# CrystalSixone/VLN-MAGIC

Hardware: AMD Instinct MI355X
Metric: trajectory-steps/sec (whole node), MAGIC-S R2R pretrain (higher is better)
Workload: dtype bf16

## Files before the change

include/magic_hip.h:

```cpp
#ifndef MAGIC_HIP_H
#define MAGIC_HIP_H
#ifdef __cplusplus
extern "C" {
#endif

#define MAGIC_OK 0
#define MAGIC_ERR_ARG (-1)
#define MAGIC_ERR_LAUNCH (-2)
#define MAGIC_ERR_UNSUPPORTED (-3)

int magic_abi_version(void);
int magic_build_id(char* out, int len);
int magic_device_info(int* cu_count, int* clock_khz, char* arch, int arch_len);

int magic_gemm(int dtype, int layout, int batch, int nh, int M, int N, int K,
               const void* A, int lda, long long sAb, long long sAh,
               const void* B, int ldb, long long sBb, long long sBh,
               void* C, int ldc, long long sCb, long long sCh, int c_f32, int accumulate,
               const float* bias, int epilogue, const void* aux, int ldaux,
               const void* residual, int ldr, void* C2, int ldc2,
               float alpha, int splitk, float* bias_grad, void* stream);
int magic_gemm_set_big(int mode);
#define MAGIC_GEMM_FORM_PLAIN 0x1
#define MAGIC_GEMM_FORM_XCD 0x2
// ... 148 lines not shown
int magic_lndot_fwd(int dtype, int M, int H, const void* Y, const float* gamma, const float* beta, float eps,
                    const float* w2, const float* b2, float* logit, void* stream);
int magic_lndot_bwd_blocks(int M);
int magic_lndot_bwd(int dtype, int M, int H, const void* Y, const float* gamma, const float* beta, float eps,
                    const float* w2, const float* dlogit, void* dZ, float* dgamma, float* dbeta, float* dw2, float* db2,
                    float* part, void* stream);

int magic_ce_rows(int dtype, int M, int N, const void* logits, int ld, const int* labels, int ignore_index,
                  float coef, const float* row_w, float* loss_row, void* dlogits, int ldd, int accumulate,
                  float* w_out, float w_rate, void* stream);
int magic_softkl_rows(int dtype, int M, int N, const void* logits, int ld, const float* targets, int ldt, float coef,
                      const float* row_w , float* loss_row, void* dlogits, int ldd,
                      void* stream);

int magic_kd_rows(int M, int N, const float* s, const float* t, int ld, float temperature, const float* w, float norm,
                  float coef, const float* coef_dev, float* loss_row, float* ds, int accumulate, void* stream);
int magic_mse(int dtype, int g_f32, long long outer, long long inner, const void* s, long long s_stride, const void* t,
              long long t_stride, const float* w, long long rows_per_w, float norm, float coef, const float* coef_dev, float* loss, void* ds,
              long long g_stride, int accumulate, void* stream);
typedef struct {
  int g_f32; long long outer, inner; const void* s; long long s_stride; const void* t; long long t_stride;
  const float* w; long long rows_per_w; float norm, coef; const float* coef_dev; float* loss; void* ds; long long g_stride; int accumulate;
  const int* valid_dev; const float* norm_dev; long long valid_mod;
} magic_mse_desc;
int magic_mse_multi(int dtype, int n, const magic_mse_desc* d, void* stream);
int magic_kd_emb_supported(int dtype, int Hs, int Ht);
int magic_kd_emb(int dtype, int n, const magic_mse_desc* d, int Hs, int Ht, const int* M, const void* const* W, const float* const* b,
                 void* const* d_acc, void* stream);
int magic_cfp_loss(int dtype, int B, int H, const void* a0, const void* a1, const void* a2, const void* txt, float temperature, float coef,
                   float* rows, void* d0, void* d1, void* d2, void* dtxt, float* part, int* counter, void* stream);

int magic_mlm_eval_supported(int dtype, int H);
int magic_mlm_eval_ws_need(int dtype, int nm, int V, int H);
int magic_mlm_eval(int dtype, int nm, int V, int H, const void* hm, const void* W, int ldw, const float* bias,
                   const int* labels, int ignore_index, void* ws, float* loss_row, int* hit_row, void* stream);
int magic_eval_rows(int dtype, int M, int N, const void* logits, int ld, const int* labels, int ignore_index,
                    const float* targets, int ldt, float* loss_row, int* hit_row, void* stream);
int magic_cfp_eval(int dtype, int B, int H, const void* a, const void* txt, float temperature,
                   float* loss_row, int* hit_row, void* stream);
int magic_eval_accum(int M, const float* loss_row, const int* hit_row, void* acc, int slot, void* stream);

int magic_csr_gather(int dtype, int n_out, int H, const void* src, const int* ptr, const int* idx, const float* w,
                     void* out, int accumulate, void* stream);
int magic_pano_fuse_fwd(int dtype, int N, int V, int H, const void* x, const int* lens, const float* wf, const float* bf,
                        void* fused, float* probs, const void* P, int nh, int inner, float* pmean, void* stream);
typedef struct {
  int B, K, Vp, use_gate;
  const float *g_raw, *l_raw, *fuse_raw; const unsigned char *gmask, *lmask; const int* fsrc; const unsigned char* bwmask;
// ... 131 lines not shown
```

vln-magic_amd/csrc/loss.hip:

```cpp
#include "common.hpp"
#include <cstdint>

static const float* g_seed_scale = nullptr;
const float* seed_scale_get() { return g_seed_scale; }
extern "C" int magic_seed_scale(const float* scale_dev) { g_seed_scale = scale_dev; return MAGIC_OK; }

template <typename T>
__global__ __launch_bounds__(256) void ce_rows_kernel(int M, int N, const T* logits, int ld, const int* labels, int ignore_index,
                                                      float coef, const float* row_w, float* loss_row, T* dlogits, int ldd,
                                                      int accumulate, float* w_out, float w_rate, const float* ss) {
  __shared__ float red[8];
  if (ss) coef *= ss[0];
  const int row = blockIdx.x, tid = threadIdx.x, lane = tid & 63, wid = tid >> 6;
  const T* x = logits + (long long)row * ld;
  const int lab = labels[row];
  const bool ignored = (lab == ignore_index) || lab < 0 || lab >= N;
  const float xl = ignored ? 0.f : to_f(x[lab]);
  float mx = -3.0e38f;
  for (int c = tid; c < N; c += 256) mx = fmaxf(mx, to_f(x[c]));
  mx = wave_max(mx);
  if (lane == 0) red[wid] = mx;
  __syncthreads();
  mx = fmaxf(fmaxf(red[0], red[1]), fmaxf(red[2], red[3]));
  __syncthreads();
// ... 191 lines not shown
  if (coef_dev) coef *= coef_dev[0];
  if (ss) coef *= ss[0];
  const long long total = outer * inner;
  float acc = 0.f;
  for (long long i = (long long)blockIdx.x * 256 + threadIdx.x; i < total; i += (long long)gridDim.x * 256) {
    const long long o = i / inner, r = i % inner;
    const float d = to_f(s[o * s_stride + r]) - to_f(t[o * t_stride + r]);
    const float wv = w ? w[o / rows_per_w] : 1.f;
    acc += wv * d * d;
    if (ds) {
      float g = 2.f * coef * norm * wv * d;
      G* p = ds + o * g_stride + r;
      if (accumulate) g += to_f(*p);
      *p = from_f<G>(g);
    }
  }
  acc = wave_sum(acc);
  if ((threadIdx.x & 63) == 0) red[threadIdx.x >> 6] = acc;
  __syncthreads();
  if (threadIdx.x == 0 && loss) atomicAdd(loss, (red[0] + red[1] + red[2] + red[3]) * norm);
}

#define MSE_MAX 10
struct MseMulti { magic_mse_desc d[MSE_MAX]; int start[MSE_MAX + 1]; int vec[MSE_MAX]; int n; const float* ss; };

#define MSE_NT 1024
template <typename T, typename G>
__device__ __forceinline__ void mse_body(const magic_mse_desc& p, int bid, int nblk, float* red, const float* ss) {
  float coef = p.coef;
  if (p.coef_dev) coef *= p.coef_dev[0];
  if (ss) coef *= ss[0];
  const T* s = (const T*)p.s; const T* t = (const T*)p.t; G* ds = (G*)p.ds;
  const long long total = p.outer * p.inner;
  const long long vo = p.valid_dev ? p.valid_dev[0] : p.outer, vi = p.valid_dev ? p.valid_dev[1] : p.inner;
  const float nrm = p.norm * (p.norm_dev ? p.norm_dev[0] : 1.f);
  float acc = 0.f;
  for (long long i = (long long)bid * MSE_NT + threadIdx.x; i < total; i += (long long)nblk * MSE_NT) {
    const long long o = i / p.inner, r = i % p.inner;
    const bool ok = o < vo && (p.valid_mod > 0 ? r % p.valid_mod : r) < vi;
    const float d = ok ? to_f(s[o * p.s_stride + r]) - to_f(t[o * p.t_stride + r]) : 0.f;
    const float wv = p.w ? p.w[o / p.rows_per_w] : 1.f;
    acc += wv * d * d;
    if (ds) {
      float g = 2.f * coef * nrm * wv * d;
      G* q = ds + o * p.g_stride + r;
      if (p.accumulate) g += to_f(*q);
      *q = from_f<G>(g);
    }
  }
  acc = wave_sum(acc);
  if ((threadIdx.x & 63) == 0) red[threadIdx.x >> 6] = acc;
  __syncthreads();
  if (threadIdx.x == 0 && p.loss) {
    float v = 0.f;
    for (int w = 0; w < MSE_NT / 64; ++w) v += red[w];
    atomicAdd(p.loss, v * nrm);
  }
}

template <typename Hh, typename G>
__device__ __forceinline__ void mse_body_v8(const magic_mse_desc& p, int bid, int nblk, float* red, const float* ss) {
  float coef = p.coef;
  if (p.coef_dev) coef *= p.coef_dev[0];
  if (ss) coef *= ss[0];
  const Hh* s = (const Hh*)p.s; const Hh* t = (const Hh*)p.t; G* ds = (G*)p.ds;
  const unsigned in8 = (unsigned)(p.inner >> 3), tot8 = (unsigned)p.outer * in8, rpw = (unsigned)p.rows_per_w;
  const unsigned stride = (unsigned)nblk * MSE_NT;
  const unsigned vo = p.valid_dev ? (unsigned)p.valid_dev[0] : (unsigned)p.outer, vi = p.valid_dev ? (unsigned)p.valid_dev[1] : (unsigned)p.inner;
  const float nrm = p.norm * (p.norm_dev ? p.norm_dev[0] : 1.f);
  const float c2 = 2.f * coef * nrm;
// ... 9 lines not shown
      ok[u] = i < tot8;
      const unsigned ii = ok[u] ? i : i0;
      o[u] = ii / in8; r[u] = (ii - o[u] * in8) << 3;
      sv[u] = *(const h16x8<Hh>*)(s + (long long)o[u] * p.s_stride + r[u]);
      tv[u] = *(const h16x8<Hh>*)(t + (long long)o[u] * p.t_stride + r[u]);
    }
#pragma unroll
    for (int u = 0; u < 2; ++u) {
      if (!ok[u]) continue;
      const float wv = p.w ? p.w[o[u] / rpw] : 1.f;
      float d[8];
      float a = 0.f;
      const unsigned rm = vm ? r[u] % vm : r[u];
#pragma unroll
      for (int e = 0; e < 8; ++e) { d[e] = (o[u] < vo && rm + e < vi) ? (float)sv[u][e] - (float)tv[u][e] : 0.f; a += d[e] * d[e]; }
      acc += wv * a;
      if (ds) {
        G* q = ds + (long long)o[u] * p.g_stride + r[u];
        const float cw = c2 * wv;
        if constexpr (sizeof(G) == 4) {
          f32x4 g0, g1;
#pragma unroll
          for (int e = 0; e < 4; ++e) { g0[e] = cw * d[e]; g1[e] = cw * d[4 + e]; }
          if (p.accumulate) { g0 += *(const f32x4*)q; g1 += *(const f32x4*)(q + 4); }
          *(f32x4*)q = g0; *(f32x4*)(q + 4) = g1;
        } else {
          h16x8<Hh> g;
          if (p.accumulate) {
            const h16x8<Hh> old = *(const h16x8<Hh>*)q;
#pragma unroll
            for (int e = 0; e < 8; ++e) g[e] = (Hh)(cw * d[e] + (float)old[e]);
          } else {
#pragma unroll
            for (int e = 0; e < 8; ++e) g[e] = (Hh)(cw * d[e]);
          }
          *(h16x8<Hh>*)q = g;
        }
      }
    }
  }
  acc = wave_sum(acc);
  if ((threadIdx.x & 63) == 0) red[threadIdx.x >> 6] = acc;
  __syncthreads();
  if (threadIdx.x == 0 && p.loss) {
    float v = 0.f;
    for (int w = 0; w < MSE_NT / 64; ++w) v += red[w];
    atomicAdd(p.loss, v * nrm);
  }
}

template <typename T>
__global__ __launch_bounds__(MSE_NT) void mse_multi_kernel(MseMulti mm) {
  __shared__ float red[MSE_NT / 64];
  int i = 0;
  while (i + 1 < mm.n && (int)blockIdx.x >= mm.start[i + 1]) ++i;
  const magic_mse_desc& p = mm.d[i];
  const int bid = blockIdx.x - mm.start[i], nblk = mm.start[i + 1] - mm.start[i];
  if constexpr (sizeof(T) == 4) mse_body<float, float>(p, bid, nblk, red, mm.ss);
  else if (p.g_f32 & 2) mse_body<float, float>(p, bid, nblk, red, mm.ss);
  else if (mm.vec[i]) { if (p.g_f32 & 1) mse_body_v8<T, float>(p, bid, nblk, red, mm.ss); else mse_body_v8<T, T>(p, bid, nblk, red, mm.ss); }
  else { if (p.g_f32 & 1) mse_body<T, float>(p, bid, nblk, red, mm.ss); else mse_body<T, T>(p, bid, nblk, red, mm.ss); }
}

#define MSE_BLOCKS 256
extern "C" int magic_mse_multi(int dtype, int n, const magic_mse_desc* d, void* stream) {
  if (n <= 0 || n > MSE_MAX || !d) return MAGIC_ERR_ARG;
  if (!dtype_ok(dtype)) return MAGIC_ERR_ARG;
  MseMulti mm;
  mm.n = n;
  mm.ss = g_seed_scale;
  long long work[MSE_MAX], all = 0;
  for (int i = 0; i < n; ++i) {
    if (d[i].outer <= 0 || d[i].inner <= 0 || !d[i].s || !d[i].t || (d[i].w && d[i].rows_per_w <= 0)) return MAGIC_ERR_ARG;
    mm.d[i] = d[i];
    const long long tot = d[i].outer * d[i].inner;
    const magic_mse_desc& q = d[i];
    const bool vec = dtype_is16(dtype) && !(q.g_f32 & 2) && tot < 0x7FFFFFFFll && q.inner % 8 == 0 && q.s_stride % 8 == 0 && q.t_stride % 8 == 0 &&
                     !((uintptr_t)q.s & 15) && !((uintptr_t)q.t & 15) && (!q.ds || (q.g_stride % 8 == 0 && !((uintptr_t)q.ds & 15))) && q.valid_mod % 8 == 0;
    mm.vec[i] = vec ? 1 : 0;
    work[i] = vec ? (tot + 7) / 8 : tot;
    all += work[i];
  }
  int total = 0;
  for (int i = 0; i < n; ++i) {
    long long blocks = (work[i] * MSE_BLOCKS + all - 1) / all;
    const long long need = (work[i] + MSE_NT - 1) / MSE_NT;
    if (blocks > need) blocks = need;
    if (blocks < 1) blocks = 1;
    mm.start[i] = total;
    total += (int)blocks;
  }
  for (int i = n; i <= MSE_MAX; ++i) mm.start[i] = total;
  dim3 grid(total), block(MSE_NT);
  hipStream_t st = (hipStream_t)stream;
  if (dtype == DT_BF16) hipLaunchKernelGGL(mse_multi_kernel<bf16>, grid, block, 0, st, mm);
  else if (dtype == DT_F16) hipLaunchKernelGGL(mse_multi_kernel<f16>, grid, block, 0, st, mm);
  else hipLaunchKernelGGL(mse_multi_kernel<float>, grid, block, 0, st, mm);
  return launch_status();
}

#define CFP_B 64
// ... 213 lines not shown
  if (seed_out) { seed_out[0] = (int)(draw(0) & 0x7FFFFFFFu); seed_out[1] = (int)(draw(1) & 0x7FFFFFFFu); }
  if (rw_out) {
    float z[5], mx = -3.0e38f;
    for (int i = 0; i < 5; ++i) {
      const float u1 = ((float)(draw(2 + 2 * i) >> 8) + 1.0f) * (1.0f / 16777217.0f);
      const float u2 = (float)(draw(3 + 2 * i) >> 8) * (1.0f / 16777216.0f);
      z[i] = sqrtf(-2.0f * logf(u1)) * cosf(6.28318530717958648f * u2) / rw_temp;
      mx = fmaxf(mx, z[i]);
    }
    float s = 0.f;
    for (int i = 0; i < 5; ++i) { z[i] = expf(z[i] - mx); s += z[i]; }
    for (int i = 0; i < 5; ++i) rw_out[i] = 5.0f * z[i] / s;
  }
}
extern "C" int magic_step_rng(unsigned long long base_seed, unsigned* counter, float rw_temp, int* seed_out, float* rw_out, float* zero_me,
                              float* scale_state, float growth, float backoff, int interval, void* stream) {
  if (!counter || rw_temp <= 0.f || (!seed_out && !rw_out)) return MAGIC_ERR_ARG;
  if (scale_state && (!(growth >= 1.f) || !(backoff > 0.f && backoff <= 1.f) || interval <= 0)) return MAGIC_ERR_ARG;
  hipLaunchKernelGGL(step_rng_kernel, dim3(1), dim3(64), 0, (hipStream_t)stream, (unsigned)base_seed, (unsigned)(base_seed >> 32), counter, rw_temp, seed_out, rw_out, zero_me,
                     scale_state, growth, backoff, interval);
  return launch_status();
}

__global__ __launch_bounds__(256) void loss_assemble_kernel(const float* rows, int n_rows, const float* row_w, float row_scale, const float* kd_rows, int n_kd,
                                                            float* slots, const float* rw, float alpha, int has_kd, float* out) {
  __shared__ float red[2][4];
  float s = 0.f, k = 0.f;
  for (int i = threadIdx.x; i < n_rows; i += 256) s += row_w ? rows[i] * row_w[i] : rows[i];
  if (kd_rows) for (int i = threadIdx.x; i < n_kd; i += 256) k += kd_rows[i];
  s = wave_sum(s); k = wave_sum(k);
  if ((threadIdx.x & 63) == 0) { red[0][threadIdx.x >> 6] = s; red[1][threadIdx.x >> 6] = k; }
  __syncthreads();
  if (threadIdx.x == 0) {
    const float sup = ((red[0][0] + red[0][1]) + (red[0][2] + red[0][3])) * row_scale;
    if (kd_rows) slots[9] = (red[1][0] + red[1][1]) + (red[1][2] + red[1][3]);
    const int ab[10] = {0, 0, 1, 1, 1, 2, 2, 3, 3, 4};
    float kdl = 0.f;
    for (int i = 0; i < 10; ++i) {
      const float t = has_kd ? slots[i] * (rw ? rw[ab[i]] : 1.f) : 0.f;
      out[1 + i] = t; kdl += t;
    }
    out[0] = sup; out[11] = kdl; out[12] = has_kd ? alpha * kdl + (1.f - alpha) * sup : sup;
  }
}
extern "C" int magic_loss_assemble(const float* rows, int n_rows, const float* row_w, float row_scale, const float* kd_rows, int n_kd,
                                   float* slots, const float* rw, float alpha, int has_kd, float* out, void* stream) {
  if (!rows || n_rows <= 0 || !out || (has_kd && !slots) || (kd_rows && n_kd <= 0)) return MAGIC_ERR_ARG;
  hipLaunchKernelGGL(loss_assemble_kernel, dim3(1), dim3(256), 0, (hipStream_t)stream, rows, n_rows, row_w, row_scale, kd_rows, n_kd, slots, rw, alpha, has_kd, out);
  return launch_status();
}
```

vln-magic_amd/host/lib.py:

```python
import ctypes as C
import os
import threading

import torch

from . import abi

_HERE = os.path.dirname(os.path.abspath(__file__))
LIB_PATH = os.environ.get("MAGIC_LIB_FILE") or os.path.join(os.path.dirname(_HERE), "libmagic_hip.so")

vp, i32, i64, f32, u32, u64 = C.c_void_p, C.c_int, C.c_longlong, C.c_float, C.c_uint, C.c_ulonglong


class MagicHipError(RuntimeError):
    pass


try:
    SIGNATURES, STRUCTS = abi.load()
except (OSError, ValueError) as e:
    raise MagicHipError(f"{abi.HEADER}: the C ABI header cannot be read ({e}); the binding has no other table") from e

DwDesc = STRUCTS["magic_dw_desc"]
DwCatProb = STRUCTS["magic_dwcat_prob"]
# ... 146 lines not shown
        e0, e1 = torch.cuda.Event(enable_timing=True), torch.cuda.Event(enable_timing=True)
        e0.record()
        rc = _fn(name)(*args)
        e1.record()
        PROFILE["events"].append((name, args[1] if name == "magic_gemm" else -1, e0, e1))
        if PROFILE.get("shapes") is not None:
            PROFILE["shapes"].append(tuple(a for a in args[:7] if isinstance(a, int) and abs(a) < (1 << 24)))
    else:
        rc = _fn(name)(*args)
    if rc != 0:
        raise MagicHipError(f"{name} failed: {_ERR.get(rc, rc)}")


class solo:

    def __enter__(self):
        self.prev = getattr(_tls, "solo", False)
        _tls.solo = True
        return self

    def __exit__(self, et, ev, tb):
        _tls.solo = self.prev
        return False


def call(name, *args):
    ls = getattr(_tls, "lockstep", None)
    if ls is not None and name in PAIRABLE and not getattr(_tls, "solo", False):
        return ls.submit(ls.index(), name, args)
    if ls is not None and PROFILE["on"]:
        with ls.cv:
            return _raw_call(name, args)
    _raw_call(name, args)


class group:

    def __enter__(self):
        self.on = getattr(_tls, "lockstep", None) is None and not _DEBUG_SYNC
        if self.on:
            if PROFILE["on"]:
                self.ev = (torch.cuda.Event(enable_timing=True), torch.cuda.Event(enable_timing=True))
                self.ev[0].record()
            if load().magic_group_begin() != 0:
                raise MagicHipError("magic_group_begin failed (nested grouping?)")
            _tls.in_group = True
# ... 222 lines not shown
```

vln-magic_amd/host/model_pretrain.py:

```python
import os

import torch
import torch.nn as nn

from . import ops as O
from .config import cfg_get
from .ddp import refuse_torch_ddp
from .engine import Ctx, MagicNet, cls_specs, rup, trunk_specs
from .params import ParamStore
from .plan import build_plan, check_plan

MID_CUT = 2
LOCKSTEP = not os.environ.get("MAGIC_NO_LOCKSTEP")
LOCKSTEP_EAGER = bool(os.environ.get("MAGIC_LOCKSTEP_EAGER"))
DYN_TERMS = ("txt_emb", "txt_attn", "img_emb", "img_fused", "img_attn", "g_emb", "g_attn", "l_emb", "l_attn")
KD_SLOTS = ("txt_emb_loss", "txt_attn_loss", "img_emb_loss", "avg_img_emb_loss", "img_attn_loss",
            "global_emb_loss", "global_attn_loss", "local_emb_loss", "local_attn_loss", "predict_loss")


PRETRAIN_CAUSAL = ("back_txt", "back_img")


def pretrain_specs(cfg):
    H = cfg.hidden_size
# ... 398 lines not shown
        i = DYN_TERMS.index(term)
        d["fill"][term] = fn
        return dict(valid_dev=d["i"][2 * i:2 * i + 2], norm_dev=d["f"][i:i + 1], norm=1.0, valid_mod=mod)

    def _kd_emb(self, c, slot, s_t, t_t, proj, M, outer, w, coef, d_acc, dyn=None):
        c.kd_emb.append((slot, s_t, t_t, self.net.lin(f"bert.{proj}.weight"), M, outer, w, coef, d_acc, dyn))

    def _kd_attn(self, c, slot, sP, tP, Bn, Nq, Nk, ldp, nh_s, nh_t, w, coef, dyn=None):
        n = self.net
        hmin = min(nh_s, nh_t)
        dP = None
        if self.store.requires_grad:
            dP = (n.new if hmin == nh_s else n.zeros)(Bn, nh_s, Nq, ldp, dtype=torch.float32)
        q = dict(s=sP, t=tP, outer=Bn, inner=hmin * Nq * ldp, s_stride=nh_s * Nq * ldp, t_stride=nh_t * Nq * ldp, w=w, rows_per_w=1,
                 norm=1.0 / (Bn * hmin * Nq * Nk), coef=coef[0], coef_dev=coef[1], loss=c.slots[slot:slot + 1], ds=dP,
                 g_stride=nh_s * Nq * ldp)
        if dyn is not None:
            term, qk, kk = dyn
            q.update(self._dyn(c, term, lambda t, Bn=Bn, hmin=hmin, Nq=Nq, Nk=Nk, ldp=ldp, qk=qk, kk=kk:
                               (Bn, (t[qk] if qk else Nq) * ldp, 1.0 / (Bn * hmin * (t[qk] if qk else Nq) * (t[kk] if kk else Nk))), mod=Nq * ldp))
        c.kd_mse.append(q)
        return dP

    def _kd_flush(self, c):
        from . import lib as L
        n, train = self.net, self.store.requires_grad
        jobs = c.kd_emb
        fused = bool(jobs) and all(
            O.kd_emb_ok(s_t.dtype, pl.K, pl.N) and t_t.dtype == s_t.dtype and s_t.is_contiguous() and t_t.is_contiguous() and pl.W.is_contiguous()
            and not ((s_t.data_ptr() | t_t.data_ptr() | pl.W.data_ptr() | (d_acc.data_ptr() if train else 0)) & 15)
            and (not train or d_acc.is_contiguous()) for (_, s_t, t_t, pl, _, _, _, _, d_acc, _) in jobs)
        sps = [None] * len(jobs)
        if not fused:
            with L.group():
                sps = [O.linear_fwd(s_t, pl.W, pl.b, M) for (_, s_t, _, pl, M, _, _, _, _, _) in jobs]
        dss, emb = [], []
        for (slot, s_t, t_t, pl, M, outer, w, coef, d_acc, dyn), sp in zip(jobs, sps):
            Ht = pl.N
            inner = (M // outer) * Ht
            ds = n.new(M, Ht) if train else None
            dss.append(ds)
            q = dict(s=sp, t=t_t, outer=outer, inner=inner, s_stride=inner, t_stride=inner, w=w, rows_per_w=1, norm=1.0 / (M * Ht),
                     coef=coef[0], coef_dev=coef[1], loss=c.slots[slot:slot + 1], ds=ds, g_stride=inner)
            if dyn is not None:
                term, ok, ik = dyn
                rows = M // outer
                q.update(self._dyn(c, term, lambda t, outer=outer, rows=rows, Ht=Ht, ok=ok, ik=ik:
                                   ((t[ok] if ok else outer), (t[ik] if ik else rows) * Ht,
                                    1.0 / ((t[ok] if ok else outer) * (t[ik] if ik else rows) * Ht))))
            if fused:
                q.pop("valid_mod", None)
                q.update(s=s_t, M=M, W=pl.W, b=pl.b, d_acc=d_acc if train else None)
                emb.append(q)
            else:
                c.kd_mse.append(q)
        if emb:
            O.kd_emb(emb)
        if c.kd_mse:
            O.mse_multi(c.kd_mse)
        if train:
            for (slot, s_t, t_t, pl, M, outer, w, coef, d_acc, dyn), ds in zip(jobs, dss):
                O.linear_dw(ds, s_t, pl.dW, pl.db, M)
            if not fused:
                with L.group():
                    for (slot, s_t, t_t, pl, M, outer, w, coef, d_acc, dyn), ds in zip(jobs, dss):
                        O.linear_dx(ds, pl.W, M, out=d_acc, residual=d_acc)
        c.kd_emb, c.kd_mse = [], []

    def _rw_device(self, rw):
        if rw is None:
            rw = [1.0] * 5
        if torch.is_tensor(rw) and rw.is_cuda:
            return rw
        cached = getattr(self, "_rwd_cache", None)
        key = tuple(float(x) for x in rw)
        if cached is None or cached[0] != key:
            self._rwd_cache = cached = (key, torch.tensor(list(key), dtype=torch.float32).to(self.device_))
        return cached[1]

    def _losses(self, c, o, t, rw):
        n, cfg, plan, task = self.net, self.config, c.plan, c.task
        B, L, K, Vp, H = plan["B"], plan["L"], plan["K"], plan["Vp"], n.H
        train = self.store.requires_grad
        O.defer_dw(train)
        kdl = getattr(cfg, "kdl", None)
        kd = t is not None and kdl is not None
        alpha = float(kdl["kd_alpha"]) if kd else 0.0
        sc = 1.0 - alpha
        dyn = train and self.loss_scale is not None
        gs = float(self.grad_scale) if (train and not dyn) else 1.0
# ... 77 lines not shown
            c.d_cls0 = (zz(B, H), zz(B, H), zz(B, H))
            temp = float(cfg_get(cfg, "cfp_temperature"))
            c.rows = n.new(6, B, dtype=torch.float32)
            txt_o = c.cfp[3]
            c.dsim, c.d_cfp = [], None
            ar = plan["arange_b"]
            lds = c.lds = rup(B, 8)
            fused = O.cfp_loss_ok(B, H)
            if fused:
                c.d_cfp = [n.new(B, H) for _ in range(4)] if train else None
                O.cfp_loss(B, H, c.cfp[:3], txt_o, temp, scg * 0.5 / B, c.rows, d_a=c.d_cfp[:3] if train else None, d_txt=c.d_cfp[3] if train else None)
            for i in (() if fused else range(3)):
                a = c.cfp[i]
                sim, simT = n.new(B, lds, dtype=torch.float32), n.new(B, lds, dtype=torch.float32)
                O.gemm(0, a, txt_o, sim, B, B, H, H, H, lds, alpha=1.0 / temp)
                O.gemm(0, txt_o, a, simT, B, B, H, H, H, lds, alpha=1.0 / temp)
                d1 = n.new(B, lds, dtype=torch.float32) if train else None
                d2 = n.new(B, lds, dtype=torch.float32) if train else None
                O.ce_rows(sim, B, B, lds, ar, coef=scg * 0.5 / B, loss_row=c.rows[2 * i], dlogits=d1, ldd=lds)
                O.ce_rows(simT, B, B, lds, ar, coef=scg * 0.5 / B, loss_row=c.rows[2 * i + 1], dlogits=d2, ldd=lds)
                c.dsim.append((d1, d2))
            c.temp = temp
            sup_rows, sup_w, sup_scale = c.rows, None, 0.5 / B
        kd_rows, rwd = None, None
        if kd:
            if rw is None:
                rw = [1.0] * 5
            rwd = self._rw_device(rw)
            rw = [(alpha * gs, rwd[i:i + 1]) for i in range(5)]
            tasks, types = kdl["kdl_tasks"], kdl["kdl_task_types"]
            emb, att = "emb" in types, "attn" in types
            T = float(kdl["kd_temperature"])
            w = None
            if kdl.get("teacher_sample_hard_mining", False) and task == "sap":
                if getattr(c, "sap_w", None) is not None:
                    w = c.sap_w
                else:
                    w = n.new(B, dtype=torch.float32)
                    O.ce_rows(t["fused_logits"], B, K, K, plan["global_act_labels"], w_out=w,
                              w_rate=float(kdl["t_sample_preprocess_exp_decay"]))
            nh_s = n.nh
            nh_t = t["txt_attns"].shape[1]
            Np, V = plan["Np"], plan["V"]
            if "txt" in tasks:
                if emb:
                    self._kd_emb(c, 0, o["txt_embeds"], t["txt_embeds"], "txt_emb_w", B * L, B, w, rw[0], c.d_txt, dyn=("txt_emb", None, "L"))
                if att:
                    c.dP_txt = self._kd_attn(c, 1, o["txt_attns"], t["txt_attns"], B, L, L, c.txt.ldp, nh_s, nh_t, w, rw[0], dyn=("txt_attn", "L", "L"))
            wp = w if (w is not None and Np == B) else None
            if "img" in tasks:
                if emb:
                    self._kd_emb(c, 2, o["pano_embeds"], t["pano_embeds"], "kdl_img_w", Np * V, Np, wp, rw[1], c.d_pano, dyn=("img_emb", "Np", None))
                    self._kd_emb(c, 3, o["pano_fused_embeds"], t["pano_fused_embeds"], "kdl_avg_img_w", Np, Np, wp, rw[1], c.d_fused, dyn=("img_fused", "Np", None))
                if att:
                    ldp = c.pano.ldp
                    g_img = n.new(Np, V, ldp, dtype=torch.float32) if train else None
                    q = dict(s=o["img_attns"], t=t["img_attns"], outer=Np, inner=V * ldp, s_stride=V * ldp, t_stride=V * ldp, w=wp, rows_per_w=1,
                             norm=1.0 / (Np * V * V), coef=rw[1][0], coef_dev=rw[1][1], loss=c.slots[4:5], ds=g_img, g_stride=V * ldp)
                    q.update(self._dyn(c, "img_attn", lambda tr, V=V, ldp=ldp: (tr["Np"], V * ldp, 1.0 / (tr["Np"] * V * V))))
                    c.kd_mse.append(q)
            if "global" in tasks and task != "mrc":
                if task == "mlm":
                    x, Pm, Nq, Nk, ldp, d_acc, qk, kk = c.l2v.out, c.l2v.P, L, K, c.l2v.ldp, c.d_x, "L", "K"
                else:
                    x, Pm, Nq, Nk, ldp, d_acc, qk, kk = c.glob.out, c.glob.P, K, L, c.glob.ldp, c.d_gmap, "K", "L"
                if emb:
                    self._kd_emb(c, 5, x, t["gmap_embeds"], "global_cross_w", B * Nq, B, w, rw[2], d_acc, dyn=("g_emb", None, qk))
                if att:
                    c.dP_g = self._kd_attn(c, 6, Pm, t["gmap_attns"], B, Nq, Nk, ldp, nh_s, nh_t, w, rw[2], dyn=("g_attn", qk, kk))
            if "local" in tasks and task != "mlm":
                if emb:
                    self._kd_emb(c, 7, c.loc.out, t["vp_embeds"], "local_cross_w", B * Vp, B, w, rw[3], c.d_vp, dyn=("l_emb", None, None))
                if att:
                    c.dP_l = self._kd_attn(c, 8, c.loc.P, t["vp_attns"], B, Vp, L, c.loc.ldp, nh_s, nh_t, w, rw[3], dyn=("l_attn", None, "L"))
            self._kd_flush(c)
            if "img" in tasks and att and train:
                c.dP_pano = n.new(Np, nh_s, V, c.pano.ldp, dtype=torch.float32)
                O.head_mean_bwd(g_img, c.dP_pano, Np, nh_s, V * c.pano.ldp)
            if "predict" in tasks and task == "sap":
                if getattr(c, "sap_fused", False):
                    kd_rows = c.kdrows
                else:
                    c.kdrows = n.new(B, dtype=torch.float32)
                    O.kd_rows(c.fl, t["fused_logits"], B, K, K, T, w=w, norm=(1.0 / B if w is not None else 1.0 / (B * K)),
                              coef=rw[4][0], coef_dev=rw[4][1], loss_row=c.kdrows, ds=c.dfl, accumulate=True)
                    kd_rows = c.kdrows
        lo = O.loss_assemble(sup_rows.reshape(-1), sup_w, sup_scale, kd_rows, c.slots, rwd, alpha, kd, n.new(16, dtype=torch.float32))
        res["supervised_loss"] = lo[0]
        if kd:
            res["kdl_terms"] = {k: lo[1 + i] for i, k in enumerate(KD_SLOTS)}
            res["kdl_loss"] = lo[11]
        res["loss"] = lo[12]
        return res

    def backward(self, on_bucket=None):
        self.backward_phase1()
        c = self._ctx
        if on_bucket is not None:
            O.flush_dw(keep_active=True)
            on_bucket(0, c)

            def cut():
                O.flush_dw(keep_active=True)
                on_bucket(1, c)
            self.backward_phase2(on_cut=cut)
            on_bucket(2, c)
        else:
            self.backward_phase2()

    @torch.no_grad()
# ... 159 lines not shown
```

vln-magic_amd/host/ops.py:

```python
import ctypes as C
import os

import torch

from . import lanes
from . import lib as L

FLOPS = {"total": 0.0, "gemm": 0.0, "linear_ln": 0.0, "attn": 0.0, "enc": 0.0, "enabled": False}
BYTES = {"dw": 0.0, "dw_launches": 0}


def _count(m, n, k, batch=1, fam="gemm"):
    if FLOPS["enabled"]:
        f = 2.0 * m * n * k * batch
        FLOPS["total"] += f
        FLOPS[fam] += f


def _chk(cond, msg):
    if not cond:
        raise L.MagicHipError("shape check failed: " + msg)


def gemm(layout, A, B, C, M, N, K, lda, ldb, ldc, *, batch=1, nh=1, sA=(0, 0), sB=(0, 0), sC=(0, 0),
# ... 917 lines not shown
def softkl_rows(logits, M, N, ld, targets, *, coef=0.0, row_w=None, loss_row=None, dlogits=None, ldd=0):
    _chk(targets.dtype == torch.float32 and targets.stride(-1) == 1, "softkl targets fp32")
    _chk(row_w is None or (row_w.dtype == torch.float32 and row_w.numel() >= M), "softkl row_w fp32 [M]")
    L.call("magic_softkl_rows", L.dt(logits.dtype), M, N, L.P(logits), ld, L.P(targets), targets.stride(0), float(coef),
           L.P(row_w), L.P(loss_row), L.P(dlogits), ldd, L.stream())


def kd_rows(s, t, M, N, ld, temperature, *, w=None, norm=1.0, coef=0.0, coef_dev=None, loss_row=None, ds=None, accumulate=False):
    _chk(s.dtype == torch.float32 and t.dtype == torch.float32, "kd logits fp32")
    L.call("magic_kd_rows", M, N, L.P(s), L.P(t), ld, float(temperature), L.P(w), float(norm), float(coef), L.P(coef_dev), L.P(loss_row),
           L.P(ds), 1 if accumulate else 0, L.stream())


def mse(s, t, outer, inner, s_stride, t_stride, *, w=None, rows_per_w=1, norm=1.0, coef=0.0, coef_dev=None, loss=None, ds=None, g_stride=0,
        accumulate=False):
    _chk(s.dtype == t.dtype, "mse dtypes")
    g_f32 = 1 if (ds is not None and ds.dtype == torch.float32) else 0
    if s.dtype == torch.float32:
        g_f32 = 1
    L.call("magic_mse", L.dt(s.dtype), g_f32, outer, inner, L.P(s), s_stride, L.P(t), t_stride, L.P(w), rows_per_w, float(norm),
           float(coef), L.P(coef_dev), L.P(loss), L.P(ds), g_stride, 1 if accumulate else 0, L.stream())


def mse_multi(problems):
    half = [q["s"].dtype for q in problems if q["s"].dtype != torch.float32]
    dt0 = half[0] if half else torch.float32
    i = 0
    while i < len(problems):
        chunk = problems[i:i + 10]
        arr = (L.MseDesc * len(chunk))()
        for j, q in enumerate(chunk):
            s_, t_, ds = q["s"], q["t"], q.get("ds")
            in32 = s_.dtype == torch.float32
            _chk(s_.dtype == t_.dtype and (in32 or s_.dtype == dt0), "mse_multi dtypes")
            _chk(not in32 or ds is None or ds.dtype == torch.float32, "mse_multi: fp32 inputs take an fp32 gradient")
            g_f32 = (3 if dt0 != torch.float32 else 1) if in32 else (1 if (ds is not None and ds.dtype == torch.float32) else 0)
            arr[j] = L.MseDesc(g_f32, q["outer"], q["inner"], L.P(s_), q["s_stride"], L.P(t_), q["t_stride"], L.P(q.get("w")),
                               q.get("rows_per_w", 1), float(q.get("norm", 1.0)), float(q.get("coef", 0.0)), L.P(q.get("coef_dev")),
                               L.P(q.get("loss")), L.P(ds), q.get("g_stride", 0), 1 if q.get("accumulate") else 0,
                               L.P(q.get("valid_dev")), L.P(q.get("norm_dev")), int(q.get("valid_mod", 0)))
        L.call("magic_mse_multi", L.dt(dt0), len(chunk), arr, L.stream())
        i += len(chunk)


KD_FUSED = not os.environ.get("MAGIC_NO_KD_FUSED")
_KDE_OK = {}


def kd_emb_ok(dtype, Hs, Ht):
    if not KD_FUSED or dtype not in L.HALF:
        return False
    key = (L.dt(dtype), int(Hs), int(Ht))
    if key not in _KDE_OK:
        _KDE_OK[key] = bool(L.load().magic_kd_emb_supported(*key))
    return _KDE_OK[key]


def kd_emb(problems):
    i = 0
    while i < len(problems):
        chunk = problems[i:i + 8]
        n = len(chunk)
        W0 = chunk[0]["W"]
# ... 264 lines not shown
def sap_fuse_bwd(B, K, Vp, g_raw, l_raw, fuse_raw, gmask, lmask, fsrc, bwmask, use_gate, dgl, dll, dfl, dg_raw, dl_raw, dfuse_raw):
    L.call("magic_sap_fuse_bwd", B, K, Vp, L.P(g_raw), L.P(l_raw), L.P(fuse_raw), L.P(gmask), L.P(lmask), L.P(fsrc), L.P(bwmask),
           1 if use_gate else 0, L.P(dgl), L.P(dll), L.P(dfl), L.P(dg_raw), L.P(dl_raw), L.P(dfuse_raw), L.stream())


def step_rng(base_seed, counter, rw_temp, seed_out=None, rw_out=None, zero_me=None, scale_state=None, growth=2.0, backoff=0.5, interval=2000):
    L.call("magic_step_rng", int(base_seed) & 0xFFFFFFFFFFFFFFFF, L.P(counter), float(rw_temp), L.P(seed_out), L.P(rw_out), L.P(zero_me),
           L.P(scale_state), float(growth), float(backoff), int(interval), L.stream())


def rowgate_fwd(mode, x, M, H, wx, *, e=None, we=None, b0=None, b1=None, out_s=None, out=None, gsave=None):
    L.call("magic_rowgate_fwd", L.dt(x.dtype), M, H, mode, L.P(x), L.P(e), L.P(wx), L.P(we), L.P(b0), L.P(b1), L.P(out_s), L.P(out), L.P(gsave), L.stream())


def rowgate_bwd(mode, x, M, H, wx, *, e=None, we=None, gsave=None, dy=None, dout=None, dx=None, de=None, dwx=None, dwe=None, db0=None, db1=None):
    L.call("magic_rowgate_bwd", L.dt(x.dtype), M, H, mode, L.P(x), L.P(e), L.P(wx), L.P(we), L.P(gsave), L.P(dy), L.P(dout), L.P(dx), L.P(de),
           L.P(dwx), L.P(dwe), L.P(db0), L.P(db1), L.stream())


def seed_scale(scale_state):
    L.call("magic_seed_scale", L.P(scale_state))


def loss_assemble(rows, row_w, row_scale, kd_rows, slots, rw, alpha, has_kd, out):
    _chk(rows.dtype == torch.float32 and rows.is_contiguous() and out.dtype == torch.float32 and out.numel() >= 13, "loss_assemble layout")
    L.call("magic_loss_assemble", L.P(rows), rows.numel(), L.P(row_w), float(row_scale), L.P(kd_rows), kd_rows.numel() if kd_rows is not None else 0,
           L.P(slots), L.P(rw), float(alpha), 1 if has_kd else 0, L.P(out), L.stream())
    return out


def sumsq(g, out):
    L.call("magic_sumsq", g.numel(), L.P(g), L.P(out), L.stream())


def sumsq_sched(g, out, step, lr0, warmup, total, b1, b2, lr_ss):
    _chk(step.numel() >= 2 and step.dtype == torch.int32, "schedule step words: int32[2] {global_step, optimizer state step}")
    L.call("magic_sumsq_sched", g.numel(), L.P(g), L.P(out), L.P(step), float(lr0), int(warmup), int(total), float(b1), float(b2), L.P(lr_ss), L.stream())


def adamw(n, p, g, m, v, shadow, lr, b1, b2, eps, wd, step_size, sumsq_buf, max_norm, gscale, lr_ss=None, n_decay=-1, zero_grad=False, overflow=None,
          scale_state=None, sched_step=None, decay_first=False):
    _chk(sched_step is None or (sched_step.numel() >= 2 and sched_step.dtype == torch.int32), "schedule step words: int32[2] {global_step, optimizer state step}")
    L.call("magic_adamw", n, L.P(p), L.P(g), L.P(m), L.P(v), L.P(shadow), L.dt(shadow.dtype) if shadow is not None else 1, float(lr), float(b1), float(b2), float(eps), float(wd),
           float(step_size), L.P(sumsq_buf), float(max_norm), float(gscale), L.P(lr_ss), int(n_decay), 1 if zero_grad else 0, L.P(overflow),
           L.P(scale_state), L.P(sched_step), 1 if decay_first else 0, L.stream())

# ... 36 lines not shown
```

Measured before the change: 197,400.

## Fuse head-plane gradient broadcast and loss assembly into the MSE multi-kernel

The multi-problem MSE kernel can now write the image-attention gradient straight into per-head fp32 planes, each divided by the head count. This replaces the separate head_mean_bwd launch and its intermediate buffer. A last-block-done atomic counter lets the final block run the loss-assembly reduction inside the same launch, removing another small kernel. The cost is a grid-wide atomic and fence on every block, extra plane stores, and tail state passed through a thread-local set before launch.

New measurement: 196,800. Within noise of the previous version (-0.3%).

```diff
diff --git a/include/magic_hip.h b/include/magic_hip.h
--- a/include/magic_hip.h
+++ b/include/magic_hip.h
@@ -194,8 +194,11 @@
   int g_f32; long long outer, inner; const void* s; long long s_stride; const void* t; long long t_stride;
   const float* w; long long rows_per_w; float norm, coef; const float* coef_dev; float* loss; void* ds; long long g_stride; int accumulate;
   const int* valid_dev; const float* norm_dev; long long valid_mod;
+  int g_planes; long long g_plane_stride;
 } magic_mse_desc;
 int magic_mse_multi(int dtype, int n, const magic_mse_desc* d, void* stream);
+int magic_mse_tail(const float* rows, int n_rows, const float* row_w, float row_scale, const float* kd_rows, int n_kd,
+                   float* slots, const float* rw, float alpha, int has_kd, float* out, int* counter);
 int magic_kd_emb_supported(int dtype, int Hs, int Ht);
 int magic_kd_emb(int dtype, int n, const magic_mse_desc* d, int Hs, int Ht, const int* M, const void* const* W, const float* const* b,
                  void* const* d_acc, void* stream);
diff --git a/profiles/micro/loss_tail_probe.py b/profiles/micro/loss_tail_probe.py
--- /dev/null
+++ b/profiles/micro/loss_tail_probe.py
@@ -0,0 +1,85 @@
+import os
+import statistics
+import sys
+
+import torch
+
+sys.path.insert(0, os.path.join(os.path.dirname(os.path.abspath(__file__)), "..", ".."))
+import magic_amd
+from magic_amd.host import ops as O
+
+ROUNDS = int(sys.argv[1]) if len(sys.argv) > 1 else 12
+REPS = int(sys.argv[2]) if len(sys.argv) > 2 else 20
+DT, NH, NHT, B, NP, V, LDP = torch.bfloat16, 2, 12, 48, 281, 36, 40
+dev = "cuda"
+slots = torch.zeros(16, device=dev)
+rw = torch.ones(5, device=dev)
+rows = torch.rand(3 * B, device=dev)
+kd_rows = torch.rand(B, device=dev)
+out = torch.empty(16, device=dev)
+probs = []
+for slot, (nq, ldp) in ((1, (80, 80)), (6, (27, 80)), (8, (37, 80))):
+    s = torch.rand(B, NH, nq, ldp, device=dev).to(DT)
+    t = torch.rand(B, NHT, nq, ldp, device=dev).to(DT)
+    probs.append(dict(s=s, t=t, outer=B, inner=NH * nq * ldp, s_stride=NH * nq * ldp, t_stride=NHT * nq * ldp, w=None, rows_per_w=1, norm=1.0 / s.numel(),
+                      coef=1.0, coef_dev=rw[0:1], loss=slots[slot:slot + 1], ds=torch.empty(B, NH, nq, ldp, device=dev), g_stride=NH * nq * ldp))
+s_img, t_img = torch.rand(NP, V, LDP, device=dev), torch.rand(NP, V, LDP, device=dev)
+g_img = torch.empty(NP, V, LDP, device=dev)
+dP = torch.empty(NP, NH, V, LDP, device=dev)
+img = dict(s=s_img, t=t_img, outer=NP, inner=V * LDP, s_stride=V * LDP, t_stride=V * LDP, w=None, rows_per_w=1, norm=1.0 / (NP * V * V), coef=1.0,
+           coef_dev=rw[1:2], loss=slots[4:5])
+asm = dict(rows=rows, row_w=None, row_scale=1.0 / B, kd_rows=kd_rows, slots=slots, rw=rw, alpha=0.5, has_kd=True, out=out)
+
+
+NEW = hasattr(O, "LOSS_TAIL")
+plain = probs[:1] + [dict(img, ds=g_img, g_stride=V * LDP)] + probs[1:]
+planes = probs[:1] + [dict(img, ds=dP, g_stride=NH * V * LDP, g_planes=NH, g_plane_stride=V * LDP)] + probs[1:]
+
+
+def mse_only():
+    O.mse_multi(plain)
+
+
+def sequence():
+    O.mse_multi(plain)
+    O.head_mean_bwd(g_img, dP, NP, NH, V * LDP)
+    O.loss_assemble(rows, None, 1.0 / B, kd_rows, slots, rw, 0.5, True, out)
+
+
+def planes_only():
+    O.mse_multi(planes)
+    O.loss_assemble(rows, None, 1.0 / B, kd_rows, slots, rw, 0.5, True, out)
+
+
+def fused():
+    O.mse_multi(planes, tail=asm)
+
+
+def timed(fn):
+    e0, e1 = torch.cuda.Event(enable_timing=True), torch.cuda.Event(enable_timing=True)
+    e0.record()
+    for _ in range(REPS):
+        fn()
+    e1.record()
+    e1.synchronize()
+    return e0.elapsed_time(e1) * 1e3 / REPS
+
+
+forms = [("mse_multi alone", mse_only), ("sequence (3 launches)", sequence)] + ([("planes + assemble (2)", planes_only), ("fused (1 launch)", fused)] if NEW else [])
+for _ in range(3):
+    for _, fn in forms:
+        fn()
+torch.cuda.synchronize()
+ts = {name: [] for name, _ in forms}
+for r in range(ROUNDS):
+    for name, fn in forms:
+        ts[name].append(timed(fn))
+print(f"attention-map terms of a sap step, B {B}, {NP} panoramas x {V} views, {NH} student heads, bf16; {ROUNDS} rounds x {REPS} back-to-back calls per form, "
+      "interleaved; us per call")
+print("round  " + "  ".join(f"{name:>22s}" for name, _ in forms))
+for r in range(ROUNDS):
+    print(f"{r:5d}  " + "  ".join(f"{ts[name][r]:22.2f}" for name, _ in forms))
+for name, _ in forms:
+    print(f"{name:22s} median {statistics.median(ts[name]):6.2f} us  min {min(ts[name]):6.2f} us")
+if NEW:
+    print(f"difference of medians, sequence - fused: {statistics.median(ts['sequence (3 launches)']) - statistics.median(ts['fused (1 launch)']):.2f} us per call")
diff --git a/vln-magic_amd/csrc/loss.hip b/vln-magic_amd/csrc/loss.hip
--- a/vln-magic_amd/csrc/loss.hip
+++ b/vln-magic_amd/csrc/loss.hip
@@ -237,7 +237,9 @@
 }
 
 #define MSE_MAX 10
-struct MseMulti { magic_mse_desc d[MSE_MAX]; int start[MSE_MAX + 1]; int vec[MSE_MAX]; int n; const float* ss; };
+struct MseTail { const float* rows; const float* row_w; const float* kd_rows; float* slots; const float* rw; float* out; int* counter;
+                 int n_rows, n_kd, has_kd; float row_scale, alpha; };
+struct MseMulti { magic_mse_desc d[MSE_MAX]; int start[MSE_MAX + 1]; int vec[MSE_MAX]; int n; const float* ss; MseTail tail; };
 
 #define MSE_NT 1024
 template <typename T, typename G>
@@ -259,8 +261,14 @@
     if (ds) {
       float g = 2.f * coef * nrm * wv * d;
       G* q = ds + o * p.g_stride + r;
-      if (p.accumulate) g += to_f(*q);
-      *q = from_f<G>(g);
+      if (sizeof(G) == 4 && p.g_planes > 1) {
+        const int nh = p.g_planes;
+        const G v = from_f<G>(g / nh);
+        for (int h = 0; h < nh; ++h) q[h * p.g_plane_stride] = v;
+      } else {
+        if (p.accumulate) g += to_f(*q);
+        *q = from_f<G>(g);
+      }
     }
   }
   acc = wave_sum(acc);
@@ -316,8 +324,15 @@
           f32x4 g0, g1;
 #pragma unroll
           for (int e = 0; e < 4; ++e) { g0[e] = cw * d[e]; g1[e] = cw * d[4 + e]; }
-          if (p.accumulate) { g0 += *(const f32x4*)q; g1 += *(const f32x4*)(q + 4); }
-          *(f32x4*)q = g0; *(f32x4*)(q + 4) = g1;
+          if (p.g_planes > 1) {
+            const int nh = p.g_planes;
+#pragma unroll
+            for (int e = 0; e < 4; ++e) { g0[e] = g0[e] / nh; g1[e] = g1[e] / nh; }
+            for (int h = 0; h < nh; ++h) { *(f32x4*)(q + h * p.g_plane_stride) = g0; *(f32x4*)(q + h * p.g_plane_stride + 4) = g1; }
+          } else {
+            if (p.accumulate) { g0 += *(const f32x4*)q; g1 += *(const f32x4*)(q + 4); }
+            *(f32x4*)q = g0; *(f32x4*)(q + 4) = g1;
+          }
         } else {
           h16x8<Hh> g;
           if (p.accumulate) {
@@ -343,9 +358,13 @@
   }
 }
 
+__device__ void loss_assemble_body(int tid, const float* rows, int n_rows, const float* row_w, float row_scale, const float* kd_rows, int n_kd,
+                                   float* slots, const float* rw, float alpha, int has_kd, float* out);
+
 template <typename T>
 __global__ __launch_bounds__(MSE_NT) void mse_multi_kernel(MseMulti mm) {
   __shared__ float red[MSE_NT / 64];
+  __shared__ int is_last;
   int i = 0;
   while (i + 1 < mm.n && (int)blockIdx.x >= mm.start[i + 1]) ++i;
   const magic_mse_desc& p = mm.d[i];
@@ -354,23 +373,48 @@
   else if (p.g_f32 & 2) mse_body<float, float>(p, bid, nblk, red, mm.ss);
   else if (mm.vec[i]) { if (p.g_f32 & 1) mse_body_v8<T, float>(p, bid, nblk, red, mm.ss); else mse_body_v8<T, T>(p, bid, nblk, red, mm.ss); }
   else { if (p.g_f32 & 1) mse_body<T, float>(p, bid, nblk, red, mm.ss); else mse_body<T, T>(p, bid, nblk, red, mm.ss); }
+  const MseTail& tl = mm.tail;
+  if (!tl.out) return;
+  if (threadIdx.x == 0) {
+    __builtin_amdgcn_fence(__ATOMIC_RELEASE, "workgroup");
+    asm volatile("s_waitcnt vmcnt(0)" ::: "memory");
+    is_last = (atomicAdd(tl.counter, 1) == (int)gridDim.x - 1) ? 1 : 0;
+  }
+  __syncthreads();
+  if (!is_last) return;
+  __builtin_amdgcn_fence(__ATOMIC_ACQUIRE, "agent");
+  loss_assemble_body(threadIdx.x, tl.rows, tl.n_rows, tl.row_w, tl.row_scale, tl.kd_rows, tl.n_kd, tl.slots, tl.rw, tl.alpha, tl.has_kd, tl.out);
+  if (threadIdx.x == 0) *tl.counter = 0;
 }
 
 #define MSE_BLOCKS 256
+static thread_local MseTail t_mse_tail = {};
+extern "C" int magic_mse_tail(const float* rows, int n_rows, const float* row_w, float row_scale, const float* kd_rows, int n_kd,
+                              float* slots, const float* rw, float alpha, int has_kd, float* out, int* counter) {
+  t_mse_tail = MseTail{};
+  if (!out) return MAGIC_OK;
+  if (!rows || n_rows <= 0 || !counter || (has_kd && !slots) || (kd_rows && (n_kd <= 0 || !slots))) return MAGIC_ERR_ARG;
+  t_mse_tail = MseTail{rows, row_w, kd_rows, slots, rw, out, counter, n_rows, n_kd, has_kd, row_scale, alpha};
+  return MAGIC_OK;
+}
 extern "C" int magic_mse_multi(int dtype, int n, const magic_mse_desc* d, void* stream) {
+  MseMulti mm;
+  mm.tail = t_mse_tail;
+  t_mse_tail = MseTail{};
   if (n <= 0 || n > MSE_MAX || !d) return MAGIC_ERR_ARG;
   if (!dtype_ok(dtype)) return MAGIC_ERR_ARG;
-  MseMulti mm;
   mm.n = n;
   mm.ss = g_seed_scale;
   long long work[MSE_MAX], all = 0;
   for (int i = 0; i < n; ++i) {
     if (d[i].outer <= 0 || d[i].inner <= 0 || !d[i].s || !d[i].t || (d[i].w && d[i].rows_per_w <= 0)) return MAGIC_ERR_ARG;
+    if (d[i].g_planes < 0 || (d[i].g_planes > 1 && (!d[i].ds || !(d[i].g_f32 & 1) || d[i].accumulate || d[i].g_plane_stride < d[i].inner))) return MAGIC_ERR_ARG;
     mm.d[i] = d[i];
     const long long tot = d[i].outer * d[i].inner;
     const magic_mse_desc& q = d[i];
     const bool vec = dtype_is16(dtype) && !(q.g_f32 & 2) && tot < 0x7FFFFFFFll && q.inner % 8 == 0 && q.s_stride % 8 == 0 && q.t_stride % 8 == 0 &&
-                     !((uintptr_t)q.s & 15) && !((uintptr_t)q.t & 15) && (!q.ds || (q.g_stride % 8 == 0 && !((uintptr_t)q.ds & 15))) && q.valid_mod % 8 == 0;
+                     !((uintptr_t)q.s & 15) && !((uintptr_t)q.t & 15) && (!q.ds || (q.g_stride % 8 == 0 && !((uintptr_t)q.ds & 15))) && q.valid_mod % 8 == 0 &&
+                     (q.g_planes <= 1 || q.g_plane_stride % 8 == 0);
     mm.vec[i] = vec ? 1 : 0;
     work[i] = vec ? (tot + 7) / 8 : tot;
     all += work[i];
@@ -630,26 +674,37 @@
   return launch_status();
 }
 
+__device__ void loss_assemble_body(int tid, const float* rows, int n_rows, const float* row_w, float row_scale, const float* kd_rows, int n_kd,
+                                   float* slots, const float* rw, float alpha, int has_kd, float* out) {
+  __shared__ float red[2][4];
+  float s = 0.f, k = 0.f, sl = 0.f, w = 1.f;
+  if (tid < 10 && has_kd) {
+    sl = __hip_atomic_load(slots + tid, __ATOMIC_RELAXED, __HIP_MEMORY_SCOPE_AGENT);
+    if (rw) w = rw[tid < 2 ? 0 : tid < 5 ? 1 : tid < 7 ? 2 : tid < 9 ? 3 : 4];
+  }
+  if (tid < 256) {
+    for (int i = tid; i < n_rows; i += 256) s += row_w ? rows[i] * row_w[i] : rows[i];
+    if (kd_rows) for (int i = tid; i < n_kd; i += 256) k += kd_rows[i];
+    s = wave_sum(s); k = wave_sum(k);
+    if ((tid & 63) == 0) { red[0][tid >> 6] = s; red[1][tid >> 6] = k; }
+  }
+  __syncthreads();
+  if (tid >= 64) return;
+  const float sup = ((red[0][0] + red[0][1]) + (red[0][2] + red[0][3])) * row_scale;
+  const float s9 = (red[1][0] + red[1][1]) + (red[1][2] + red[1][3]);
+  if (kd_rows && tid == 9) sl = s9;
+  const float t = has_kd ? sl * w : 0.f;
+  if (tid < 10) out[1 + tid] = t;
+  float kdl = 0.f;
+  for (int i = 0; i < 10; ++i) kdl += __shfl(t, i);
+  if (tid == 0) {
+    if (kd_rows) slots[9] = s9;
+    out[0] = sup; out[11] = kdl; out[12] = has_kd ? alpha * kdl + (1.f - alpha) * sup : sup;
+  }
+}
 __global__ __launch_bounds__(256) void loss_assemble_kernel(const float* rows, int n_rows, const float* row_w, float row_scale, const float* kd_rows, int n_kd,
                                                             float* slots, const float* rw, float alpha, int has_kd, float* out) {
-  __shared__ float red[2][4];
-  float s = 0.f, k = 0.f;
-  for (int i = threadIdx.x; i < n_rows; i += 256) s += row_w ? rows[i] * row_w[i] : rows[i];
-  if (kd_rows) for (int i = threadIdx.x; i < n_kd; i += 256) k += kd_rows[i];
-  s = wave_sum(s); k = wave_sum(k);
-  if ((threadIdx.x & 63) == 0) { red[0][threadIdx.x >> 6] = s; red[1][threadIdx.x >> 6] = k; }
-  __syncthreads();
-  if (threadIdx.x == 0) {
-    const float sup = ((red[0][0] + red[0][1]) + (red[0][2] + red[0][3])) * row_scale;
-    if (kd_rows) slots[9] = (red[1][0] + red[1][1]) + (red[1][2] + red[1][3]);
-    const int ab[10] = {0, 0, 1, 1, 1, 2, 2, 3, 3, 4};
-    float kdl = 0.f;
-    for (int i = 0; i < 10; ++i) {
-      const float t = has_kd ? slots[i] * (rw ? rw[ab[i]] : 1.f) : 0.f;
-      out[1 + i] = t; kdl += t;
-    }
-    out[0] = sup; out[11] = kdl; out[12] = has_kd ? alpha * kdl + (1.f - alpha) * sup : sup;
-  }
+  loss_assemble_body(threadIdx.x, rows, n_rows, row_w, row_scale, kd_rows, n_kd, slots, rw, alpha, has_kd, out);
 }
 extern "C" int magic_loss_assemble(const float* rows, int n_rows, const float* row_w, float row_scale, const float* kd_rows, int n_kd,
                                    float* slots, const float* rw, float alpha, int has_kd, float* out, void* stream) {
diff --git a/vln-magic_amd/host/lib.py b/vln-magic_amd/host/lib.py
--- a/vln-magic_amd/host/lib.py
+++ b/vln-magic_amd/host/lib.py
@@ -192,6 +192,12 @@
     def __exit__(self, et, ev, tb):
         _tls.solo = self.prev
         return False
+
+
+def host_call(name, *args):
+    rc = _fn(name)(*args)
+    if rc != 0:
+        raise MagicHipError(f"{name} failed: {_ERR.get(rc, rc)}")
 
 
 def call(name, *args):
diff --git a/vln-magic_amd/host/model_pretrain.py b/vln-magic_amd/host/model_pretrain.py
--- a/vln-magic_amd/host/model_pretrain.py
+++ b/vln-magic_amd/host/model_pretrain.py
@@ -444,7 +444,7 @@
         c.kd_mse.append(q)
         return dP
 
-    def _kd_flush(self, c):
+    def _kd_flush(self, c, tail=None):
         from . import lib as L
         n, train = self.net, self.store.requires_grad
         jobs = c.kd_emb
@@ -478,8 +478,9 @@
                 c.kd_mse.append(q)
         if emb:
             O.kd_emb(emb)
+        rode = tail is not None and 0 < len(c.kd_mse) <= 10
         if c.kd_mse:
-            O.mse_multi(c.kd_mse)
+            O.mse_multi(c.kd_mse, tail=tail if rode else None)
         if train:
             for (slot, s_t, t_t, pl, M, outer, w, coef, d_acc, dyn), ds in zip(jobs, dss):
                 O.linear_dw(ds, s_t, pl.dW, pl.db, M)
@@ -488,6 +489,7 @@
                     for (slot, s_t, t_t, pl, M, outer, w, coef, d_acc, dyn), ds in zip(jobs, dss):
                         O.linear_dx(ds, pl.W, M, out=d_acc, residual=d_acc)
         c.kd_emb, c.kd_mse = [], []
+        return rode
 
     def _rw_device(self, rw):
         if rw is None:
@@ -611,7 +613,7 @@
                 c.dsim.append((d1, d2))
             c.temp = temp
             sup_rows, sup_w, sup_scale = c.rows, None, 0.5 / B
-        kd_rows, rwd = None, None
+        kd_rows, rwd, tail, rode, lo = None, None, None, False, None
         if kd:
             if rw is None:
                 rw = [1.0] * 5
@@ -643,9 +645,14 @@
                     self._kd_emb(c, 3, o["pano_fused_embeds"], t["pano_fused_embeds"], "kdl_avg_img_w", Np, Np, wp, rw[1], c.d_fused, dyn=("img_fused", "Np", None))
                 if att:
                     ldp = c.pano.ldp
-                    g_img = n.new(Np, V, ldp, dtype=torch.float32) if train else None
+                    planes = train and O.LOSS_TAIL and n.dtype in O.L.HALF
+                    if planes:
+                        c.dP_pano = n.new(Np, nh_s, V, ldp, dtype=torch.float32)
+                    g_img = n.new(Np, V, ldp, dtype=torch.float32) if (train and not planes) else None
                     q = dict(s=o["img_attns"], t=t["img_attns"], outer=Np, inner=V * ldp, s_stride=V * ldp, t_stride=V * ldp, w=wp, rows_per_w=1,
                              norm=1.0 / (Np * V * V), coef=rw[1][0], coef_dev=rw[1][1], loss=c.slots[4:5], ds=g_img, g_stride=V * ldp)
+                    if planes:
+                        q.update(ds=c.dP_pano, g_stride=nh_s * V * ldp, g_planes=nh_s, g_plane_stride=V * ldp)
                     q.update(self._dyn(c, "img_attn", lambda tr, V=V, ldp=ldp: (tr["Np"], V * ldp, 1.0 / (tr["Np"] * V * V))))
                     c.kd_mse.append(q)
             if "global" in tasks and task != "mrc":
@@ -662,8 +669,13 @@
                     self._kd_emb(c, 7, c.loc.out, t["vp_embeds"], "local_cross_w", B * Vp, B, w, rw[3], c.d_vp, dyn=("l_emb", None, None))
                 if att:
                     c.dP_l = self._kd_attn(c, 8, c.loc.P, t["vp_attns"], B, Vp, L, c.loc.ldp, nh_s, nh_t, w, rw[3], dyn=("l_attn", None, "L"))
-            self._kd_flush(c)
-            if "img" in tasks and att and train:
+            pred = "predict" in tasks and task == "sap"
+            lo = n.new(16, dtype=torch.float32)
+            if O.LOSS_TAIL and n.dtype in O.L.HALF and (not pred or getattr(c, "sap_fused", False)):
+                tail = dict(rows=sup_rows.reshape(-1), row_w=sup_w, row_scale=sup_scale, kd_rows=c.kdrows if pred else None, slots=c.slots, rw=rwd,
+                            alpha=alpha, has_kd=kd, out=lo)
+            rode = self._kd_flush(c, tail)
+            if "img" in tasks and att and train and g_img is not None:
                 c.dP_pano = n.new(Np, nh_s, V, c.pano.ldp, dtype=torch.float32)
                 O.head_mean_bwd(g_img, c.dP_pano, Np, nh_s, V * c.pano.ldp)
             if "predict" in tasks and task == "sap":
@@ -674,7 +686,8 @@
                     O.kd_rows(c.fl, t["fused_logits"], B, K, K, T, w=w, norm=(1.0 / B if w is not None else 1.0 / (B * K)),
                               coef=rw[4][0], coef_dev=rw[4][1], loss_row=c.kdrows, ds=c.dfl, accumulate=True)
                     kd_rows = c.kdrows
-        lo = O.loss_assemble(sup_rows.reshape(-1), sup_w, sup_scale, kd_rows, c.slots, rwd, alpha, kd, n.new(16, dtype=torch.float32))
+        if not rode:
+            lo = O.loss_assemble(sup_rows.reshape(-1), sup_w, sup_scale, kd_rows, c.slots, rwd, alpha, kd, lo if lo is not None else n.new(16, dtype=torch.float32))
         res["supervised_loss"] = lo[0]
         if kd:
             res["kdl_terms"] = {k: lo[1 + i] for i, k in enumerate(KD_SLOTS)}
diff --git a/vln-magic_amd/host/ops.py b/vln-magic_amd/host/ops.py
--- a/vln-magic_amd/host/ops.py
+++ b/vln-magic_amd/host/ops.py
@@ -963,7 +963,12 @@
            float(coef), L.P(coef_dev), L.P(loss), L.P(ds), g_stride, 1 if accumulate else 0, L.stream())
 
 
-def mse_multi(problems):
+LOSS_TAIL = not os.environ.get("MAGIC_NO_LOSS_TAIL")
+_TAIL_COUNTER = {}
+
+
+def mse_multi(problems, tail=None):
+    _chk(tail is None or len(problems) <= 10, "mse_multi: a tail rides in ONE launch")
     half = [q["s"].dtype for q in problems if q["s"].dtype != torch.float32]
     dt0 = half[0] if half else torch.float32
     i = 0
@@ -976,10 +981,16 @@
             _chk(s_.dtype == t_.dtype and (in32 or s_.dtype == dt0), "mse_multi dtypes")
             _chk(not in32 or ds is None or ds.dtype == torch.float32, "mse_multi: fp32 inputs take an fp32 gradient")
             g_f32 = (3 if dt0 != torch.float32 else 1) if in32 else (1 if (ds is not None and ds.dtype == torch.float32) else 0)
+            nh, ps = int(q.get("g_planes", 0)), int(q.get("g_plane_stride", 0))
+            if nh > 1:
+                _chk(ds is not None and ds.dtype == torch.float32 and not q.get("accumulate") and ps >= q["inner"] and
+                     ds.numel() >= (q["outer"] - 1) * q["g_stride"] + (nh - 1) * ps + q["inner"], "mse_multi head planes")
             arr[j] = L.MseDesc(g_f32, q["outer"], q["inner"], L.P(s_), q["s_stride"], L.P(t_), q["t_stride"], L.P(q.get("w")),
                                q.get("rows_per_w", 1), float(q.get("norm", 1.0)), float(q.get("coef", 0.0)), L.P(q.get("coef_dev")),
                                L.P(q.get("loss")), L.P(ds), q.get("g_stride", 0), 1 if q.get("accumulate") else 0,
-                               L.P(q.get("valid_dev")), L.P(q.get("norm_dev")), int(q.get("valid_mod", 0)))
+                               L.P(q.get("valid_dev")), L.P(q.get("norm_dev")), int(q.get("valid_mod", 0)), nh, ps)
+        if tail is not None:
+            _mse_tail(**tail)
         L.call("magic_mse_multi", L.dt(dt0), len(chunk), arr, L.stream())
         i += len(chunk)
 
@@ -1290,6 +1301,16 @@
     L.call("magic_seed_scale", L.P(scale_state))
 
 
+def _mse_tail(rows, row_w, row_scale, kd_rows, slots, rw, alpha, has_kd, out):
+    _chk(rows.dtype == torch.float32 and rows.is_contiguous() and out.dtype == torch.float32 and out.numel() >= 13, "loss_assemble layout")
+    _chk(not has_kd or (slots is not None and slots.dtype == torch.float32 and slots.numel() >= 10), "loss_assemble slots")
+    cnt = _TAIL_COUNTER.get(out.device)
+    if cnt is None:
+        cnt = _TAIL_COUNTER[out.device] = torch.zeros(1, dtype=torch.int32, device=out.device)
+    L.host_call("magic_mse_tail", L.P(rows), rows.numel(), L.P(row_w), float(row_scale), L.P(kd_rows), kd_rows.numel() if kd_rows is not None else 0,
+                L.P(slots), L.P(rw), float(alpha), 1 if has_kd else 0, L.P(out), L.P(cnt))
+
+
 def loss_assemble(rows, row_w, row_scale, kd_rows, slots, rw, alpha, has_kd, out):
     _chk(rows.dtype == torch.float32 and rows.is_contiguous() and out.dtype == torch.float32 and out.numel() >= 13, "loss_assemble layout")
     L.call("magic_loss_assemble", L.P(rows), rows.numel(), L.P(row_w), float(row_scale), L.P(kd_rows), kd_rows.numel() if kd_rows is not None else 0,
```
